# joyfang1106/MRLA

Hardware: AMD Instinct MI355X
Metric: images/sec fwd+bwd resnet50_mrlal b=256 (higher is better)
Workload: dtype bf16

## Files before the change

include/mrla_hip.h:

```cpp
#ifndef MRLA_HIP_H_
#define MRLA_HIP_H_

#include <stddef.h>
#include <stdint.h>

#ifdef __cplusplus
extern "C" {
#endif

#define MRLA_OK 0
#define MRLA_EINVAL (-1)
#define MRLA_EUNSUPPORTED (-2)
#define MRLA_EHIP (-3)

enum { MRLA_F32 = 0, MRLA_BF16 = 1, MRLA_F16 = 2 };
enum { MRLA_NCHW = 0, MRLA_NHWC = 1 };
enum { MRLA_ACT_NONE = 0, MRLA_ACT_GELU = 1 };
enum { MRLA_BN_NONE = 0, MRLA_BN_TRAIN = 1, MRLA_BN_EVAL = 2 };

#define MRLA_FWD_MOMENTS 8
#define MRLA_BWD_MOMENTS 3
#define MRLA_GEMM_MOMENTS 4

#define MRLA_ABI_VERSION 5
// ... 196 lines not shown

int mrla_conv1x1_fwd_affine_supported(int m, int k, int n, int dtype);
int mrla_conv1x1_fwd_affine(const void* x, const void* w, const float* sc, const float* sh, int relu, void* y, int m, int k,
                            int n, int dtype, void* stream);

int mrla_conv1x1_wgrad_rows(int m, int k, int n, int dtype);
int mrla_conv1x1_wgrad_plan(int m, int k, int n, int dtype, int* out);
int mrla_conv1x1_wgrad(const void* dy, const void* x, float* part, void* dw, int m, int k, int n, int dtype, int dw_dtype,
                       void* stream);

int mrla_conv1x1_wgrad_bn_supported(int m, int k, int n, int dtype);
int mrla_conv1x1_wgrad_bn(const void* g, const void* xb, const float* sc, const float* sh, const float* cb , int relu,
                          void* dy_out, const void* x, float* part, void* dw, int m, int k, int n, int dtype, int dw_dtype,
                          void* stream);

int mrla_weight_bank_refresh(const void* table, int entries, int max_tiles, void* stream);
int mrla_weight_bank_refresh_dt(const void* table, int entries, int max_tiles, int dtype, void* stream);

int mrla_reduce_rows(const float* in, float* out, int rows, int n, void* stream);
int mrla_reduce_rows2(const float* in1, float* out1, int rows1, int n1, const float* in2, float* out2, int rows2, int n2,
                      void* stream);



int mrla_light_tail_fwd(const void* x, const float* pre_sc, const float* pre_sh, const void* o_prev, const float* wq,
                        const float* wk, int ksize, const float* wv, const float* lam, const float* gamma,
                        const float* beta, float* running_mean, float* running_var, int bn_mode, float momentum, float eps,
                        const float* dp, float* mom, void* x_out, float* gate, float* bnbuf, void* out, int b, int c,
                        int h, int w, int d, int res, int fuse, int dtype, int layout, int act, void* stream);

// ... 53 lines not shown
```

mrla_amd/_lib.py:

```python
import ctypes
import os

_HERE = os.path.dirname(os.path.abspath(__file__))
LIB_PATH = os.environ.get("MRLA_HIP_LIB") or os.path.join(_HERE, "libmrla_hip.so")

ABI_VERSION = 5
OK, EINVAL, EUNSUPPORTED, EHIP = 0, -1, -2, -3
F32, BF16, F16 = 0, 1, 2
NCHW, NHWC = 0, 1
ACT_NONE, ACT_GELU = 0, 1
BN_NONE, BN_TRAIN, BN_EVAL = 0, 1, 2
FWD_MOMENTS, BWD_MOMENTS, TOKEN_PARTIALS, GEMM_MOMENTS = 8, 3, 15, 4

_ERR = {EINVAL: "invalid argument", EUNSUPPORTED: "unsupported shape/layout for the HIP kernels",
        EHIP: "HIP runtime error at kernel launch"}

_P, _I, _F = ctypes.c_void_p, ctypes.c_int, ctypes.c_float

SIGNATURES = {
    "mrla_abi_version": [],
    "mrla_light_wgrad_rows": [_I] * 6,
    "mrla_light_stats_fwd": [_P, _P, _P, _P, _I, _I, _I, _I, _I, _I, _I, _P],
    "mrla_light_gate_fwd": [_P, _P, _P, _I, _P, _I, _I, _I, _I, _P],
    "mrla_light_bn_fwd": [_P, _P, _P, _P, _P, _P, _P, _I, _F, _F, _P, _P, _P, _P, _I, _I, _I, _I, _P],
# ... 59 lines not shown
    "mrla_bn_gate_bwd": [_P, _P, _P, _P, _P, _P] + [_I] * 6 + [_P],
    "mrla_conv1x1_rows": [_I] * 4,
    "mrla_conv1x1_plan": [_I, _I, _I, _I, _I, _P],
    "mrla_conv1x1_wgrad_plan": [_I, _I, _I, _I, _P],
    "mrla_conv1x1_fwd": [_P, _P, _P, _P, _I, _I, _I, _I, _P],
    "mrla_conv1x1_add_supported": [_I] * 4,
    "mrla_conv1x1_fwd_add": [_P, _P, _P, _P, _I, _I, _I, _I, _P],
    "mrla_conv1x1_addend_supported": [_I] * 6,
    "mrla_conv1x1_fwd_addend": [_P, _P, _P, _P] + [_I] * 9 + [_P],
    "mrla_conv1x1_fwd_affine_supported": [_I] * 4,
    "mrla_conv1x1_fwd_affine": [_P, _P, _P, _P, _I, _P, _I, _I, _I, _I, _P],
    "mrla_conv1x1_wgrad_rows": [_I] * 4,
    "mrla_conv1x1_wgrad": [_P, _P, _P, _P, _I, _I, _I, _I, _I, _P],
    "mrla_conv1x1_wgrad_bn_supported": [_I] * 4,
    "mrla_conv1x1_wgrad_bn": [_P, _P, _P, _P, _P, _I, _P, _P, _P, _P, _I, _I, _I, _I, _I, _P],
    "mrla_weight_bank_refresh": [_P, _I, _I, _P],
    "mrla_weight_bank_refresh_dt": [_P, _I, _I, _I, _P],
    "mrla_reduce_rows": [_P, _P, _I, _I, _P],
    "mrla_reduce_rows2": [_P, _P, _I, _I, _P, _P, _I, _I, _P],
    "mrla_light_tail_fwd": [_P] * 6 + [_I] + [_P] * 6 + [_I, _F, _F] + [_P] * 6 + [_I] * 10 + [_P],
    "mrla_light_tail_bwd": [_P] * 5 + [_I] + [_P] * 7 + [_I] + [_P] * 5 + [_I] + [_P] * 8 + [_I] * 10 + [_P],
    "mrla_bn_fwd": [_P, _P, _I, _P, _P, _I, _P, _P, _P, _P, _I, _F, _F, _P, _I, _P] + [_I] * 6 + [_P],
    "mrla_bn_bwd": [_P] * 5 + [_I] * 4 + [_P, _P] + [_I] * 6 + [_P],
    "mrla_stem_fwd": [_P, _P, _P, _I, _P, _P, _P, _P, _I, _F, _F, _P, _P] + [_I] * 6 + [_P],
    "mrla_stem_bwd": [_P] * 5 + [_I, _I, _P, _P] + [_I] * 6 + [_P],
    "mrla_base_layer_fwd": [_P] * 6 + [_I] + [_P] * 5 + [_I, _F, _F] + [_P] * 9 + [_I] + [_P, _P] + [_I] * 9 + [_P],
    "mrla_base_layer_bwd": ([_P] * 5 + [_I] + [_P] * 6 + [_I] + [_P] * 6 + [_I] + [_P, _P] + [_I] + [_P] * 5 + [_I] + [_P] * 5
                            + [_I] * 12 + [_P]),
    "mrla_token_light_fwd": [_P] * 8 + [_I] + [_P, _P] + [_F] + [_P] * 4 + [_I] * 6 + [_P],
    "mrla_token_light_bwd": [_P] * 10 + [_I] + [_P] * 6 + [_I] + [_P] * 6 + [_I] * 6 + [_P],
# ... 52 lines not shown
```

mrla_amd/csrc/capi.hip:

```cpp
#include <algorithm>
#include <atomic>
#include <mutex>

#include "mrla_device.h"
#include "mrla_kernels.h"

namespace mrla {

hipError_t lds_opt_in(const void* kernel, size_t bytes) {
  if (bytes <= 48 * 1024) return hipSuccess;
  constexpr unsigned kSlots = 1024;
  static std::atomic<uintptr_t> keys[kSlots];
  static std::atomic<int> granted[kSlots];
  static std::mutex raise_mutex;
  int dev = 0;
  if (hipGetDevice(&dev) != hipSuccess) return hipErrorInvalidDevice;
  const uintptr_t key = reinterpret_cast<uintptr_t>(kernel) ^ ((uintptr_t)(dev + 1) << 52);
  unsigned i = (unsigned)((key >> 4) * 0x9E3779B1u) % kSlots;
  int slot = -1;
  for (unsigned probe = 0; probe < kSlots; ++probe, i = (i + 1) % kSlots) {
    uintptr_t k = keys[i].load(std::memory_order_acquire);
    if (k == 0 && keys[i].compare_exchange_strong(k, key, std::memory_order_acq_rel)) k = key;
    if (k == key) { slot = (int)i; break; }
  }
// ... 716 lines not shown

int mrla_conv1x1_wgrad_bn(const void* g, const void* xb, const float* sc, const float* sh, const float* cb, int relu,
                          void* dy_out, const void* x, float* part, void* dw, int m, int k, int n, int dtype, int dw_dtype,
                          void* stream) {
  if (!g || !xb || !sc || !sh || !cb || !dy_out || !x || !part || !dw || m <= 0 || k <= 0 || n <= 0 || bad_dtype(dtype))
    return MRLA_EINVAL;
  if (dw_dtype != MRLA_BF16 && dw_dtype != MRLA_F16 && dw_dtype != MRLA_F32) return MRLA_EINVAL;
  if ((dw_dtype == MRLA_F16 && dtype != MRLA_F16) || (dw_dtype == MRLA_BF16 && dtype == MRLA_F16)) return MRLA_EINVAL;
  if (dtype != MRLA_BF16 && dtype != MRLA_F16) return MRLA_EUNSUPPORTED;
  if (((uintptr_t)sc | (uintptr_t)sh | (uintptr_t)cb) & 15) return MRLA_EINVAL;
  if (dy_out == g || dy_out == xb) return MRLA_EINVAL;
  return launch_conv1x1_wgrad_bn(g, xb, sc, sh, cb, relu, dy_out, x, part, dw, dw_dtype == MRLA_F32, m, k, n, dtype,
                                 (hipStream_t)stream);
}

int mrla_weight_bank_refresh(const void* table, int entries, int max_tiles, void* stream) {
  if (!table || entries <= 0 || max_tiles <= 0) return MRLA_EINVAL;
  return launch_weight_bank_refresh((const long long*)table, entries, max_tiles, MRLA_BF16, (hipStream_t)stream);
}

int mrla_weight_bank_refresh_dt(const void* table, int entries, int max_tiles, int dtype, void* stream) {
  if (!table || entries <= 0 || max_tiles <= 0 || bad_dtype(dtype)) return MRLA_EINVAL;
  if (dtype != MRLA_BF16 && dtype != MRLA_F16) return MRLA_EUNSUPPORTED;
  return launch_weight_bank_refresh((const long long*)table, entries, max_tiles, dtype, (hipStream_t)stream);
}

int mrla_reduce_rows(const float* in, float* out, int rows, int n, void* stream) {
  if (!in || !out || rows <= 0 || n <= 0) return MRLA_EINVAL;
  return launch_reduce_rows(in, out, rows, n, (hipStream_t)stream);
}
// ... 71 lines not shown
```

mrla_amd/csrc/conv1x1_wgrad.hip:

```cpp
#include <algorithm>
#include <type_traits>

#include "conv1x1_elem.h"
#include "mrla_device.h"
#include "mrla_kernels.h"

namespace mrla {
namespace {

typedef short wg_s16x4 __attribute__((ext_vector_type(4)));
typedef c1_f32x16 wg_f32x16;
typedef __attribute__((address_space(3))) wg_s16x4* lds_s16x4_ptr;

constexpr int kPC = 32;
constexpr int kWgStages = 4;
constexpr int kWgWaves = 4;
#define MRLA_WG_FLAGS 0x00020000
constexpr int kWgTarget = 256;

template <int TN, int TK, int PC>
struct WgGeo {
  static constexpr int WN = (TN >= 256 && TK <= 64) ? 4 : (TK >= 256 && TN <= 64) ? 1 : 2;
  static constexpr int WK = kWgWaves / WN;
  static constexpr int WTN = TN / WN, WTK = TK / WK;
// ... 32 lines not shown
template <typename T>
__device__ __forceinline__ typename Elem16<T>::x8 frag_value(const Frag& f) {
  return __builtin_bit_cast(typename Elem16<T>::x8, __builtin_shufflevector(f.lo, f.hi, 0, 1, 2, 3, 4, 5, 6, 7));
}
__device__ __forceinline__ unsigned wg_lds_addr(const void* p) {
  return (unsigned)(size_t)((__attribute__((address_space(3))) const char*)p);
}

struct WgBnArgs {
  const void* xb;
  const float *cb, *sc, *sh;
  void* dy_out;
  int relu;
};

__device__ __forceinline__ void wg_read16(u32x4& v, unsigned addr) {
  asm volatile("ds_read_b128 %0, %1" : "=&v"(v) : "v"(addr));
}
template <int OFF>
__device__ __forceinline__ void wg_read16_at(u32x4& v, unsigned addr) {
  asm volatile("ds_read_b128 %0, %1 offset:%2" : "=&v"(v) : "v"(addr), "n"(OFF));
}
__device__ __forceinline__ void wg_write16(unsigned addr, const u32x4& v) {
  asm volatile("ds_write_b128 %0, %1" ::"v"(addr), "v"(v) : "memory");
}
__device__ __forceinline__ void wg_fence16(u32x4& v, bool wait) {
  if (wait) asm volatile("s_waitcnt lgkmcnt(0)" : "+v"(v) : : "memory");
  else asm volatile("" : "+v"(v) : : "memory");
}

template <typename T, int TN, int TK, int ST, int PC, bool BN>
__device__ __forceinline__ void conv1x1_wgrad_body(const T* __restrict__ dY, const T* __restrict__ X,
                                                   float* __restrict__ part, int M, int N, int K, int chunks_per_wg,
                                                   int nsplits, const WgBnArgs& bn) {
#if defined(__HIP_DEVICE_COMPILE__)
  typedef WgGeo<TN, TK, PC> G;
  constexpr int CPRY = TN / 8, CPRX = TK / 8;
  constexpr int SB = G::SB + (BN ? G::YB : 0);
  static_assert(G::SB < 65536, "ds offset field");
  extern __shared__ __align__(16) unsigned char smem_raw[];
  const int lane = threadIdx.x & (kWave - 1);
  const int wave = __builtin_amdgcn_readfirstlane(threadIdx.x / kWave);
  const int tiles_k = K / TK, tiles = (N / TN) * tiles_k;
  const int per = gridDim.x >> 3;
  const int vid = (blockIdx.x & 7) * per + (blockIdx.x >> 3);
  if (vid >= tiles * nsplits) return;
  const int split = vid / tiles, tile = vid - split * tiles;
  const int tn = tile / tiles_k, tk = tile - tn * tiles_k;
  const int n0 = tn * TN, k0 = tk * TK;
  const int chunks_total = (M + PC - 1) / PC;
  const int c_begin = split * chunks_per_wg;
  const int nch = min(chunks_per_wg, chunks_total - c_begin);

  const auto rsY = __builtin_amdgcn_make_buffer_rsrc(const_cast<T*>(dY), 0, (int)((size_t)M * N * 2), MRLA_WG_FLAGS);
// ... 64 lines not shown
    for (int q = 0; q < 6; ++q) {
      const float4 v = c4[q];
      cbv[4 * q] = v.x; cbv[4 * q + 1] = v.y; cbv[4 * q + 2] = v.z; cbv[4 * q + 3] = v.w;
    }
#pragma unroll
    for (int q = 0; q < 2; ++q) {
      const float4 u = s4[q], v = h4[q];
      scv[4 * q] = u.x; scv[4 * q + 1] = u.y; scv[4 * q + 2] = u.z; scv[4 * q + 3] = u.w;
      shv[4 * q] = v.x; shv[4 * q + 1] = v.y; shv[4 * q + 2] = v.z; shv[4 * q + 3] = v.w;
    }
#pragma unroll
    for (int q = 0; q < 24; ++q) asm volatile("" : "+v"(cbv[q]));
#pragma unroll
    for (int q = 0; q < 8; ++q) asm volatile("" : "+v"(scv[q]), "+v"(shv[q]));
  }
  const int relu = BN ? bn.relu : 0;
  auto rewrite = [&](unsigned sbo) {
    u32x4 gq[G::NIY], xq[G::NIY];
    const unsigned at = lds0 + sbo + wave * 1024 + lane * 16;
#pragma unroll
    for (int i = 0; i < G::NIY; ++i) {
      wg_read16(gq[i], at + i * (kWgWaves * 1024));
      wg_read16_at<G::SB>(xq[i], at + i * (kWgWaves * 1024));
    }
#pragma unroll
    for (int i = 0; i < G::NIY; ++i) {
      wg_fence16(gq[i], i == 0);
      wg_fence16(xq[i], false);
    }
#pragma unroll
// ... 5 lines not shown
      for (int w = 0; w < 4; ++w) {
        const float gv[2] = {Elem16<T>::lo(gq[i][w]), Elem16<T>::hi(gq[i][w])};
        const float xv[2] = {Elem16<T>::lo(xq[i][w]), Elem16<T>::hi(xq[i][w])};
        float y[2];
#pragma unroll
        for (int e = 0; e < 2; ++e) {
          const int j = 2 * w + e;
          const float z = fmaf(scv[j], xv[e], shv[j]);
          const float dz = (!relu || z > 0.f) ? gv[e] : 0.f;
          y[e] = fmaf(cbv[3 * j], dz, fmaf(cbv[3 * j + 1], xv[e], cbv[3 * j + 2]));
          if constexpr (!std::is_same<T, bf16_t>::value) y[e] = as_f32_result(y[e]);
        }
        o[w] = live ? Elem16<T>::pack(y[0], y[1]) : 0u;
      }
      wg_write16(at + i * (kWgWaves * 1024), o);
      __builtin_amdgcn_raw_buffer_store_b128(o, rsO, (live ? off : 0x80000000u) | skill, 0, 0);
    }
    toff += advY;
    asm volatile("s_waitcnt lgkmcnt(0)" ::: "memory");
  };

  constexpr int KSN = PC / 16, NF = 2 * (G::BN + G::BK), NI = (BN ? 2 : 1) * G::NIY + G::NIX;
  constexpr int W_NEXT = (ST - 3) * NI + (BN && ST > 3 ? G::NIY : 0);
  static_assert(KSN % 2 == 0 && ST >= 3 && W_NEXT < 64 && (ST - 2) * NI < 64, "fragment double buffer / stages / vmcnt immediate");
  Frag fa[2][G::BN], fb[2][G::BK];
  auto read_step = [&](int buf, unsigned sbo, int ks) {
#pragma unroll
    for (int i = 0; i < G::BN; ++i) frag_issue<CPRY>(fa[buf][i], offA[i] + sbo + ks * 16 * CPRY * 16);
#pragma unroll
    for (int j = 0; j < G::BK; ++j) frag_issue<CPRX>(fb[buf][j], offB[j] + sbo + ks * 16 * CPRX * 16);
  };
  auto mfma_step = [&](int buf) {
#pragma unroll
    for (int i = 0; i < G::BN; ++i)
#pragma unroll
      for (int j = 0; j < G::BK; ++j)
        Elem16<T>::mfma(acc[i][j], frag_value<T>(fa[buf][i]), frag_value<T>(fb[buf][j]));
  };
#pragma unroll
  for (int j = 0; j < ST - 1; ++j) issue(j);
  asm volatile("s_waitcnt vmcnt(%0)" ::"n"((ST - 2) * NI) : "memory");
  if constexpr (BN) rewrite(0);
  __builtin_amdgcn_s_barrier();
  asm volatile("" ::: "memory");
  read_step(0, 0, 0);
  int stage = 0, nxt = ST - 1;
  for (int c = 0; c < nch; ++c) {
    const unsigned sbo = stage * SB;
    stage = stage + 1 == ST ? 0 : stage + 1;
#pragma unroll
    for (int ks = 0; ks < KSN; ++ks) {
      const int cur = ks & 1;
      int pending = NF;
      if (ks + 1 < KSN) {
        read_step(cur ^ 1, sbo, ks + 1);
      } else if (c + 1 < nch) {
        asm volatile("s_waitcnt vmcnt(%0)" ::"n"(W_NEXT) : "memory");
        if constexpr (BN) rewrite(stage * SB);
        __builtin_amdgcn_s_barrier();
        asm volatile("" ::: "memory");
        issue(nxt);
        nxt = nxt + 1 == ST ? 0 : nxt + 1;
        read_step(0, stage * SB, 0);
      } else {
        pending = 0;
      }
#pragma unroll
      for (int i = 0; i < G::BN; ++i) {
        if (pending) frag_fence<NF>(fa[cur][i], i == 0); else frag_fence<0>(fa[cur][i], i == 0);
      }
#pragma unroll
      for (int j = 0; j < G::BK; ++j) frag_fence<0>(fb[cur][j], false);
      mfma_step(cur);
    }
  }

  float* po = part + ((size_t)split * N + n0 + wn * G::WTN) * K + k0 + wk * G::WTK + (lane & 31);
  const int h = lane >> 5;
#pragma unroll
  for (int i = 0; i < G::BN; ++i)
#pragma unroll
    for (int j = 0; j < G::BK; ++j)
#pragma unroll
      for (int e = 0; e < 16; ++e)
        po[(size_t)(i * 32 + 8 * (e >> 2) + 4 * h + (e & 3)) * K + j * 32] = acc[i][j][e];
#endif
}

template <int TN, int TK, int ST, int PC>
// ... 12 lines not shown
}
template <int TN, int TK, int ST, int PC>
__global__ __launch_bounds__(kWgWaves* kWave) void conv1x1_wgrad_bn_kernel(const bf16_t* __restrict__ g,
                                                                           const bf16_t* __restrict__ X,
                                                                           float* __restrict__ part, int M, int N, int K,
                                                                           int chunks_per_wg, int nsplits, WgBnArgs bn) {
  conv1x1_wgrad_body<bf16_t, TN, TK, ST, PC, true>(g, X, part, M, N, K, chunks_per_wg, nsplits, bn);
}
template <int TN, int TK, int ST, int PC>
__global__ __launch_bounds__(kWgWaves* kWave) void conv1x1_wgrad_bn_f16_kernel(const f16_t* __restrict__ g,
                                                                               const f16_t* __restrict__ X,
                                                                               float* __restrict__ part, int M, int N,
                                                                               int K, int chunks_per_wg, int nsplits,
                                                                               WgBnArgs bn) {
  conv1x1_wgrad_body<f16_t, TN, TK, ST, PC, true>(g, X, part, M, N, K, chunks_per_wg, nsplits, bn);
}

template <typename TO>
__device__ __forceinline__ void conv1x1_wgrad_reduce_body(const float* __restrict__ part, TO* __restrict__ dW, int splits,
                                                          int NK) {
  __shared__ float4 red[16][16];
  const int q = threadIdx.x & 15, g = threadIdx.x >> 4;
  const int e = blockIdx.x * 64 + q * 4;
  const float4* src = reinterpret_cast<const float4*>(part + e);
  const size_t pitch = (size_t)NK / 4;
  float4 a = {0.f, 0.f, 0.f, 0.f}, b = a;
  int s = g;
  for (; s + 16 < splits; s += 32) {
    const float4 u = src[(size_t)s * pitch], v = src[(size_t)(s + 16) * pitch];
    a.x += u.x; a.y += u.y; a.z += u.z; a.w += u.w;
// ... 64 lines not shown
    return MRLA_OK;
  }
  const size_t lds = (size_t)ST * G::SB;
  if (dtype == MRLA_F16) {
    if (lds_opt_in(reinterpret_cast<const void*>(conv1x1_wgrad_f16_kernel<TN, TK, ST, PC>), lds) != hipSuccess) return MRLA_EHIP;
    hipLaunchKernelGGL((conv1x1_wgrad_f16_kernel<TN, TK, ST, PC>), grid, block, lds, st, (const f16_t*)dy, (const f16_t*)x, part,
                       M, N, K, p.chunks_per_wg, p.splits);
  } else {
    if (lds_opt_in(reinterpret_cast<const void*>(conv1x1_wgrad_kernel<TN, TK, ST, PC>), lds) != hipSuccess) return MRLA_EHIP;
    hipLaunchKernelGGL((conv1x1_wgrad_kernel<TN, TK, ST, PC>), grid, block, lds, st, (const bf16_t*)dy, (const bf16_t*)x, part,
                       M, N, K, p.chunks_per_wg, p.splits);
  }
  return MRLA_OK;
}

}

int conv1x1_wgrad_rows(int M, int K, int N) {
  const WgPlan p = wgrad_plan(M, K, N);
  return p.tiles ? p.splits : MRLA_EUNSUPPORTED;
}

int conv1x1_wgrad_plan(int M, int K, int N, int* out) {
  const WgPlan p = wgrad_plan(M, K, N);
  if (!p.tiles) return MRLA_EUNSUPPORTED;
  out[0] = p.chunks_per_wg; out[1] = kWgStages; out[2] = p.tn; out[3] = p.tk; out[4] = p.splits; out[5] = p.tiles;
  return MRLA_OK;
}

int conv1x1_wgrad_bn_supported(int M, int K, int N) {
  const WgPlan p = wgrad_plan(M, K, N);
  if (!p.tiles) return MRLA_EUNSUPPORTED;
  const int ktiles = K / p.tk;
  return ktiles == 1 || (ktiles == 2 && N <= 512) ? 1 : MRLA_EUNSUPPORTED;
}

static int launch_wgrad(const void* dy, const void* x, float* part, void* dw, int dw_f32, int M, int K, int N, int dtype,
                        hipStream_t st, const WgBnArgs* bn) {
  const WgPlan p = wgrad_plan(M, K, N);
  if (!p.tiles || (dtype != MRLA_BF16 && dtype != MRLA_F16)) return MRLA_EUNSUPPORTED;
  int rc = MRLA_EUNSUPPORTED;
#define MRLA_WG_TILE(A, B) \
  if (p.tn == A && p.tk == B) rc = launch_tile<A, B, kWgStages, kPC>(p, dy, x, part, M, K, N, dtype, st, bn);
  MRLA_WG_TILE(64, 64) MRLA_WG_TILE(64, 128) MRLA_WG_TILE(64, 256) MRLA_WG_TILE(128, 64) MRLA_WG_TILE(128, 128)
  MRLA_WG_TILE(128, 256) MRLA_WG_TILE(256, 64) MRLA_WG_TILE(256, 128)
#undef MRLA_WG_TILE
  if (rc != MRLA_OK) return rc;
  const int NK = N * K;
  if (dw_f32)
    hipLaunchKernelGGL(conv1x1_wgrad_reduce_kernel<float>, dim3(NK / 64), dim3(256), 0, st, part, (float*)dw, p.splits, NK);
  else if (dtype == MRLA_F16)
    hipLaunchKernelGGL(conv1x1_wgrad_reduce_f16_kernel, dim3(NK / 64), dim3(256), 0, st, part, (f16_t*)dw, p.splits, NK);
  else
    hipLaunchKernelGGL(conv1x1_wgrad_reduce_kernel<bf16_t>, dim3(NK / 64), dim3(256), 0, st, part, (bf16_t*)dw, p.splits, NK);
  return hip_status(hipGetLastError());
}

int launch_conv1x1_wgrad(const void* dy, const void* x, float* part, void* dw, int dw_f32, int M, int K, int N, int dtype,
                         hipStream_t st) {
  return launch_wgrad(dy, x, part, dw, dw_f32, M, K, N, dtype, st, nullptr);
}

int launch_conv1x1_wgrad_bn(const void* g, const void* xb, const float* sc, const float* sh, const float* cb, int relu,
                            void* dy_out, const void* x, float* part, void* dw, int dw_f32, int M, int K, int N, int dtype,
                            hipStream_t st) {
  if (conv1x1_wgrad_bn_supported(M, K, N) != 1) return MRLA_EUNSUPPORTED;
  const WgBnArgs bn{xb, cb, sc, sh, dy_out, relu};
  return launch_wgrad(g, x, part, dw, dw_f32, M, K, N, dtype, st, &bn);
}

}
```

mrla_amd/csrc/mrla_kernels.h:

```cpp
#pragma once
#include <hip/hip_runtime.h>
#include <stddef.h>
#include <stdint.h>

#include "../../include/mrla_hip.h"

namespace mrla {

constexpr int kMaxTasksPerWave = 4;

struct SlabGeo {
  int B, C, H, W, HW;
  int CP;
  int slabs;
  int WS;
  int PW;
  int NG;
  int NB;
  int RB;
  int BG;
  int astride;
};

inline size_t dtype_size(int dtype) { return dtype == MRLA_F32 ? 4 : 2; }
// ... 156 lines not shown
int conv1x1_kstream_stages(int M, int K, int N);
int conv1x1_kstream_rows(int M, int K, int N);
int launch_conv1x1_kstream(const void* x, const void* w, void* y, float* part, int M, int K, int N, int dtype, hipStream_t st);
int launch_conv1x1_kstream_addend(const void* x, const void* w, const void* addend, void* y, int M, int K, int N, int b, int h,
                                  int wd, int sh, int sw, int dtype, hipStream_t st);
int launch_conv1x1_kstream_affine(const void* x, const void* w, const float* sc, const float* sh, int relu, void* y, int M,
                                  int K, int N, int dtype, hipStream_t st);
int conv1x1_wgrad_rows(int M, int K, int N);
int conv1x1_wgrad_plan(int M, int K, int N, int* out);
int launch_conv1x1_wgrad(const void* dy, const void* x, float* part, void* dw, int dw_f32, int M, int K, int N, int dtype,
                         hipStream_t st);
int conv1x1_wgrad_bn_supported(int M, int K, int N);
int launch_conv1x1_wgrad_bn(const void* g, const void* xb, const float* sc, const float* sh, const float* cb, int relu,
                            void* dy_out, const void* x, float* part, void* dw, int dw_f32, int M, int K, int N, int dtype,
                            hipStream_t st);
int launch_weight_bank_refresh(const long long* table, int entries, int max_tiles, int dtype, hipStream_t st);
int launch_light_stats_fwd_wide(const void* x, const void* o, const float* wv, float* mom, void* xout, const float* psc,
                                const float* psh, void* vout, int B, int C, int H, int W, int dtype, int act,
                                hipStream_t st, bool fused_no_x = false, int mom_ranges = 1);
int launch_light_apply_fwd_wide(const void* x, const void* o, const float* wv, const float* gate, const float* sc,
                                const float* sh, const float* lam, const float* dp, void* out, int B, int C, int H,
                                int W, int d, int res, int dtype, int act, hipStream_t st);
int launch_light_apply_fwd_pre_wide(const void* pre, const void* o, const float* psc, const float* psh, const float* wv,
                                    const float* gate, const float* sc, const float* sh, const float* lam,
                                    const float* dp, void* out, int B, int C, int H, int W, int d, int res, int dtype,
                                    hipStream_t st);
int launch_light_apply_bwd_wide(const void* dout, const void* x, const void* o, const float* wv, const float* gate,
                                const float* cb, const float* lam, const float* dp, const float* dyx, void* dx,
                                void* dprev, float* dwv_part, const void* pre, const float* pre_center, float* pre_tmom,
                                int B, int C, int H, int W, int d, int res, int relu, int dtype, int act, hipStream_t st);
// ... 49 lines not shown
```

mrla_amd/functional.py:

```python
import contextlib
import ctypes
import threading
import weakref
from math import log

import torch

from . import _lib as L

_DT = {torch.float32: L.F32, torch.bfloat16: L.BF16, torch.float16: L.F16}


def k_size_for(c):
    t = int(abs((log(c, 2) + 1) / 2.0))
    return t if t % 2 else t + 1


class KernelTimer:

    def __init__(self, names=None):
        self.names = None if names is None else set(names)
        self.records = []

    def summary(self):
# ... 7 lines not shown
            d["bytes_path"] += path
        return out


TIMER = None
SEQUENCES = True


LEAN = False


SHORTCUT_ADDEND = True


WGRAD_BN = True


CHANNEL_GATE = True


EVAL_FOLD = True


def _seq():
    return SEQUENCES and TIMER is None


def _seq_call(name, *args):
    L.call(name, *args)

# ... 1449 lines not shown
    def set_materialize_grads(self, flag):
        pass

    def save_for_backward(self, *tensors):
        self.saved_tensors = tensors

    def mark_non_differentiable(self, *tensors):
        pass


class _ConvBnFn(torch.autograd.Function):

    @staticmethod
    @_on_device
    def forward(ctx, x, w, gamma, beta, running_mean, running_var, training, momentum, eps, relu, defer, box, passthrough,
                w16, w16t, sub):
        ctx.set_materialize_grads(False)
        ca, cb = _SubCtx(), _SubCtx()
        res = _Conv1x1Fn.apply(x, w, bool(training), passthrough, w16, w16t, sub)
        n, k = w.shape[0], x.shape[1]
        ca.sub = tuple(sub) if (passthrough and sub is not None) else None
        ca.wshape, ca.wstride, ca.wdtype = w.shape, w.stride(), w.dtype
        ca.saved_tensors = (x, w16 if w16 is not None else w.reshape(n, k).contiguous(), w16t)
        y, part = res[0], res[1]
        out = _BnActFn.forward(cb, y, gamma, beta, running_mean, running_var, training, momentum, eps, relu, defer,
                               part if part.numel() else None, box)
        ctx.save_for_backward(*ca.saved_tensors, *cb.saved_tensors)
        ca.saved_tensors = cb.saved_tensors = ()
        ctx.ca, ctx.cb, ctx.defer, ctx.nthrough = ca, cb, bool(defer), len(res) - 2
        if defer:
            ctx.mark_non_differentiable(out[1])
            return (y, out[1]) + tuple(res[2:])
# ... 5 lines not shown
        saved = ctx.saved_tensors
        ca, cb = ctx.ca, ctx.cb
        ca.saved_tensors, cb.saved_tensors = saved[:3], saved[3:]
        try:
            return _ConvBnFn._backward(ctx, dy, rest, saved)
        finally:
            ca.saved_tensors = cb.saved_tensors = ()

    @staticmethod
    def _backward(ctx, dy, rest, saved):
        d_through = rest[-1] if ctx.nthrough else None
        ca, cb = ctx.ca, ctx.cb
        ca.needs_input_grad = (ctx.needs_input_grad[0], ctx.needs_input_grad[1])
        x, w, _ = saved[:3]
        y, gamma32, bnbuf = saved[3:]
        tail = (None,) * 12
        if dy is None:
            gx = _Conv1x1Fn.backward(ca, None, None, d_through)[0]
            return (gx, None, None, None) + tail
        n, k = w.shape
        b, _, h, wd = x.shape
        m = b * h * wd
        lib, dt = L.load(), _DT[x.dtype]
        g = dy if dy.is_contiguous(memory_format=_CL) else None
        fused = (WGRAD_BN and TIMER is None and ctx.needs_input_grad[1] and g is not None and g.dtype == y.dtype
                 and g.data_ptr() % 16 == 0 and cb.layout == L.NHWC and w.dtype == x.dtype
                 and ca.wdtype in (x.dtype, torch.float32) and lib.mrla_conv1x1_wgrad_bn_supported(m, k, n, dt) == 1)
        if not fused:
            dyc, dgamma, dbeta = _BnActFn.backward(cb, dy)[:3]
            gx, gw = _Conv1x1Fn.backward(ca, dyc, None, d_through)[:2]
            return (gx, gw, dgamma, dbeta) + tail
# ... 6 lines not shown
            tmom = torch.empty((rows, n, 2), dtype=torch.float32, device=dev)
        small = torch.empty((5, n), dtype=torch.float32, device=dev)
        mode = L.BN_TRAIN if cb.training else L.BN_EVAL
        if SEQUENCES:
            _seq_call("mrla_bn_bwd", _ptr(g), _ptr(y), _ptr(gamma32), _ptr(bnbuf), _ptr(tmom), rows, int(handed is not None),
                      mode, cb.relu, _ptr(small), None, b, n, h, wd, dt, L.NHWC, st)
        else:
            if handed is None:
                L.call("mrla_bn_plane_dmoments", _ptr(g), _ptr(y), _ptr(bnbuf[0]), _ptr(bnbuf[1]), _ptr(bnbuf[2]), cb.relu,
                       _ptr(tmom), b, n, h, wd, dt, L.NHWC, st)
            L.call("mrla_bn_stats_bwd", _ptr(tmom), _ptr(gamma32), _ptr(bnbuf[2]), _ptr(bnbuf[3]), mode, 1, _ptr(small),
                   _ptr(small[3]), _ptr(small[4]), rows, n, m // rows, st)
        prow = lib.mrla_conv1x1_wgrad_rows(m, k, n, dt)
        part = torch.empty((prow, n, k), dtype=torch.float32, device=dev)
        gw = torch.empty((n, k), dtype=ca.wdtype, device=dev)
        dyc = torch.empty_like(y)
        L.call("mrla_conv1x1_wgrad_bn", _ptr(g), _ptr(y), _ptr(bnbuf[0]), _ptr(bnbuf[1]), _ptr(small), cb.relu, _ptr(dyc),
               _ptr(x), _ptr(part), _ptr(gw), m, k, n, dt, _DT[ca.wdtype], st)
        ca.needs_input_grad = (ctx.needs_input_grad[0], False)
        gx = _Conv1x1Fn.backward(ca, dyc, None, d_through)[0]
        gw = _grad_like(gw, ca.wshape, ca.wstride)
        return (gx, gw, small[3].to(cb.gdtype), small[4].to(cb.gdtype)) + tail


def _conv_bn_fused(conv, bn, x, fused_bn):
    if not (WGRAD_BN and TIMER is None and fused_bn and torch.is_grad_enabled() and conv.weight.requires_grad):
        return False
    if x.dtype != torch.bfloat16:
        return False
    b, k, h, w = x.shape
# ... 66 lines not shown
    return tuple(downsample[0].stride)


def _gemm_weights(conv, x):
    wt, w16, w16t = conv.weight, None, None
    if wt.dtype != x.dtype:
        book = current_bookkeeping()
        held = book.bank.get(conv, x.dtype) if (book is not None and book.bank is not None and wt.dtype == torch.float32) else None
        if held is not None:
            w16, w16t = held
        else:
            wt = wt.to(x.dtype)
    return wt, w16, w16t


def conv_bn_act(x, conv, bn, relu, defer=False, passthrough=False, subsample=None, presampled=False):
    def second(t):
        return _SubsampleFn.apply(t, subsample[0], subsample[1]) if subsample is not None else t

    fused_bn = (type(bn) is torch.nn.BatchNorm2d and bn.affine and bn.track_running_stats)
    strided = (_strided_1x1(conv) and not passthrough and x.dim() == 4
               and conv1x1_applies(conv, x, "pre" if presampled else True))
    if strided or conv1x1_applies(conv, x):
        if strided and not presampled:
            x = _SubsampleFn.apply(x, conv.stride[0], conv.stride[1])
        wt, w16, w16t = _gemm_weights(conv, x)
        if _eval_fold_applies(conv, bn, x, fused_bn, defer):
            out = _conv_bn_eval_fold(x.detach(), w16 if w16 is not None else wt, bn, relu)
            return (out, second(x)) if passthrough else out
        if _conv_bn_fused(conv, bn, x, fused_bn):
            training = bn.training
            momentum = bump_batch_counter(bn) if training else bn.momentum
            box = _DeferredBnBox() if defer else None
            through = passthrough and x.requires_grad
            res = _ConvBnFn.apply(x, wt, bn.weight, bn.bias, bn.running_mean, bn.running_var, training, momentum or 0.0,
                                  bn.eps, relu, defer, box, through, w16, w16t, subsample if through else None)
            res = res if isinstance(res, tuple) else (res,)
            out = res[0]
            if defer:
                out._mrla_affine = (res[1][0], res[1][1])
                out._mrla_bn_box = box
            if not passthrough:
                return out
            return out, (res[-1] if through else second(x))
        if passthrough and torch.is_grad_enabled() and x.requires_grad:
            y, part, through = _Conv1x1Fn.apply(x, wt, bool(fused_bn and bn.training), True, w16, w16t, subsample)
            return bn_act(y, bn, relu, defer, pre_moments=part if part.numel() else None), through
        y, part = _Conv1x1Fn.apply(x, wt, bool(fused_bn and bn.training), False, w16, w16t)
        out = bn_act(y, bn, relu, defer, pre_moments=part if part.numel() else None)
        return (out, second(x)) if passthrough else out
    if presampled:
# ... 28 lines not shown
```

mrla_amd/resnet.py:

```python

import torch
import torch.nn as nn
import torch.nn.functional as F

from . import functional as F_
from . import layers


def _conv3x3(cin, cout, stride=1, groups=1, dilation=1):
    return nn.Conv2d(cin, cout, 3, stride=stride, padding=dilation, groups=groups, bias=False, dilation=dilation)


def _conv1x1(cin, cout, stride=1):
    return nn.Conv2d(cin, cout, 1, stride=stride, bias=False)


class se_layer(nn.Module):

    def __init__(self, channel, reduction=16):
        super().__init__()
        self.avg_pool = nn.AdaptiveAvgPool2d(1)
        self.fc = nn.Sequential(nn.Linear(channel, channel // reduction, bias=False), nn.ReLU(inplace=True),
                                nn.Linear(channel // reduction, channel, bias=False), nn.Sigmoid())

# ... 37 lines not shown
        self.eca = eca_layer(planes * self.expansion, int(ECA_size)) if ECA_size is not None else None
        self._norm = norm_layer

    def trunk_pre(self, x, defer_bn3=False):
        sub = F_.shortcut_subsample(self.downsample, x)
        out, identity = F_.conv_bn_act(x, self.conv1, self.bn1, relu=True, passthrough=True, subsample=sub)
        out = F_.bn_act(self.conv2(out), self.bn2, relu=True)
        if self.se is not None or self.eca is not None:
            out = F_.conv_bn_gate(out, self.conv3, self.bn3, self.se, self.eca)
        else:
            if callable(defer_bn3):
                b_, _, h_, w_ = out.shape
                cl = out.is_contiguous(memory_format=torch.channels_last) and not out.is_contiguous()
                defer_bn3 = defer_bn3(torch.empty((b_, self.conv3.out_channels, h_, w_), dtype=out.dtype, device="meta",
                                                  memory_format=torch.channels_last if cl else torch.contiguous_format))
            out = F_.conv_bn_act(out, self.conv3, self.bn3, relu=False, defer=defer_bn3)
        if self.downsample is not None:
            ds = self.downsample
            if isinstance(ds, nn.Sequential) and len(ds) == 2 and isinstance(ds[0], nn.Conv2d):
                identity = F_.conv_bn_act(identity, ds[0], ds[1], relu=False, presampled=sub is not None)
            else:
                identity = ds(identity)
        return out, identity

    def trunk(self, x):
        out, identity = self.trunk_pre(x)
        out += identity
        return self.relu(out), identity


class MRLA_Bottleneck(_BottleneckTrunk):

    def __init__(self, inplanes, planes, stride=1, downsample=None, SE=False, ECA_size=None, groups=1, base_width=64,
                 dilation=1, norm_layer=nn.BatchNorm2d, drop_path=0.0):
        super().__init__(inplanes, planes, stride, downsample, SE, ECA_size, groups, base_width, dilation, norm_layer)
# ... 258 lines not shown
```

Measured before the change: 8749.

## Fuse the 1x1 conv dX GEMM into the BN-backward wgrad kernel

After: 8933 (median of 6 runs). 1.02x the previous value.

```diff
diff --git a/include/mrla_hip.h b/include/mrla_hip.h
--- a/include/mrla_hip.h
+++ b/include/mrla_hip.h
@@ -234,6 +234,11 @@
                           void* dy_out, const void* x, float* part, void* dw, int m, int k, int n, int dtype, int dw_dtype,
                           void* stream);
 
+int mrla_conv1x1_wgrad_bn_dx_supported(int m, int k, int n, int dtype);
+int mrla_conv1x1_wgrad_bn_dx(const void* g, const void* xb, const float* sc, const float* sh, const float* cb ,
+                             int relu, const void* x, const void* wt , void* dx , float* part, void* dw,
+                             int m, int k, int n, int dtype, int dw_dtype, void* stream);
+
 int mrla_weight_bank_refresh(const void* table, int entries, int max_tiles, void* stream);
 int mrla_weight_bank_refresh_dt(const void* table, int entries, int max_tiles, int dtype, void* stream);
 
diff --git a/mrla_amd/_lib.py b/mrla_amd/_lib.py
--- a/mrla_amd/_lib.py
+++ b/mrla_amd/_lib.py
@@ -97,6 +97,8 @@
     "mrla_conv1x1_wgrad": [_P, _P, _P, _P, _I, _I, _I, _I, _I, _P],
     "mrla_conv1x1_wgrad_bn_supported": [_I] * 4,
     "mrla_conv1x1_wgrad_bn": [_P, _P, _P, _P, _P, _I, _P, _P, _P, _P, _I, _I, _I, _I, _I, _P],
+    "mrla_conv1x1_wgrad_bn_dx_supported": [_I] * 4,
+    "mrla_conv1x1_wgrad_bn_dx": [_P, _P, _P, _P, _P, _I, _P, _P, _P, _P, _P, _I, _I, _I, _I, _I, _P],
     "mrla_weight_bank_refresh": [_P, _I, _I, _P],
     "mrla_weight_bank_refresh_dt": [_P, _I, _I, _I, _P],
     "mrla_reduce_rows": [_P, _P, _I, _I, _P],
diff --git a/mrla_amd/csrc/capi.hip b/mrla_amd/csrc/capi.hip
--- a/mrla_amd/csrc/capi.hip
+++ b/mrla_amd/csrc/capi.hip
@@ -754,6 +754,26 @@
                                  (hipStream_t)stream);
 }
 
+int mrla_conv1x1_wgrad_bn_dx_supported(int m, int k, int n, int dtype) {
+  if (m <= 0 || k <= 0 || n <= 0 || bad_dtype(dtype)) return MRLA_EINVAL;
+  if (dtype != MRLA_BF16 && dtype != MRLA_F16) return MRLA_EUNSUPPORTED;
+  return conv1x1_wgrad_bn_dx_supported(m, k, n);
+}
+
+int mrla_conv1x1_wgrad_bn_dx(const void* g, const void* xb, const float* sc, const float* sh, const float* cb, int relu,
+                             const void* x, const void* wt, void* dx, float* part, void* dw, int m, int k, int n, int dtype,
+                             int dw_dtype, void* stream) {
+  if (!g || !xb || !sc || !sh || !cb || !x || !wt || !dx || !part || !dw || m <= 0 || k <= 0 || n <= 0 || bad_dtype(dtype))
+    return MRLA_EINVAL;
+  if (dw_dtype != MRLA_BF16 && dw_dtype != MRLA_F16 && dw_dtype != MRLA_F32) return MRLA_EINVAL;
+  if ((dw_dtype == MRLA_F16 && dtype != MRLA_F16) || (dw_dtype == MRLA_BF16 && dtype == MRLA_F16)) return MRLA_EINVAL;
+  if (dtype != MRLA_BF16 && dtype != MRLA_F16) return MRLA_EUNSUPPORTED;
+  if (((uintptr_t)sc | (uintptr_t)sh | (uintptr_t)cb | (uintptr_t)wt | (uintptr_t)dx) & 15) return MRLA_EINVAL;
+  if (dx == g || dx == xb || dx == x) return MRLA_EINVAL;
+  return launch_conv1x1_wgrad_bn_dx(g, xb, sc, sh, cb, relu, x, wt, dx, part, dw, dw_dtype == MRLA_F32, m, k, n, dtype,
+                                    (hipStream_t)stream);
+}
+
 int mrla_weight_bank_refresh(const void* table, int entries, int max_tiles, void* stream) {
   if (!table || entries <= 0 || max_tiles <= 0) return MRLA_EINVAL;
   return launch_weight_bank_refresh((const long long*)table, entries, max_tiles, MRLA_BF16, (hipStream_t)stream);
diff --git a/mrla_amd/csrc/conv1x1_wgrad.hip b/mrla_amd/csrc/conv1x1_wgrad.hip
--- a/mrla_amd/csrc/conv1x1_wgrad.hip
+++ b/mrla_amd/csrc/conv1x1_wgrad.hip
@@ -70,6 +70,12 @@
   int relu;
 };
 
+struct WgDxArgs {
+  const void* wt;
+  void* dx;
+};
+constexpr int kDxRowB = 64 * 2 + 16;
+
 __device__ __forceinline__ void wg_read16(u32x4& v, unsigned addr) {
   asm volatile("ds_read_b128 %0, %1" : "=&v"(v) : "v"(addr));
 }
@@ -85,15 +91,16 @@
   else asm volatile("" : "+v"(v) : : "memory");
 }
 
-template <typename T, int TN, int TK, int ST, int PC, bool BN>
+template <typename T, int TN, int TK, int ST, int PC, bool BN, bool DX = false>
 __device__ __forceinline__ void conv1x1_wgrad_body(const T* __restrict__ dY, const T* __restrict__ X,
                                                    float* __restrict__ part, int M, int N, int K, int chunks_per_wg,
-                                                   int nsplits, const WgBnArgs& bn) {
+                                                   int nsplits, const WgBnArgs& bn, const WgDxArgs& dxa = WgDxArgs{}) {
 #if defined(__HIP_DEVICE_COMPILE__)
   typedef WgGeo<TN, TK, PC> G;
   constexpr int CPRY = TN / 8, CPRX = TK / 8;
   constexpr int SB = G::SB + (BN ? G::YB : 0);
   static_assert(G::SB < 65536, "ds offset field");
+  static_assert(!DX || (BN && TN == 256 && TK == 64 && PC == 32), "the dX form: one 256 x 64 tile");
   extern __shared__ __align__(16) unsigned char smem_raw[];
   const int lane = threadIdx.x & (kWave - 1);
   const int wave = __builtin_amdgcn_readfirstlane(threadIdx.x / kWave);
@@ -188,6 +195,19 @@
 #pragma unroll
     for (int q = 0; q < 8; ++q) asm volatile("" : "+v"(scv[q]), "+v"(shv[q]));
   }
+  u32x4 wa[DX ? 16 : 1];
+  const auto rsD = __builtin_amdgcn_make_buffer_rsrc(DX ? dxa.dx : nullptr, 0, DX ? (int)((size_t)M * K * 2) : 0, MRLA_WG_FLAGS);
+  const unsigned dlimit = (unsigned)((size_t)M * K * 2);
+  const int dr = lane & 31, dh = lane >> 5, dblk = wave & 1;
+  unsigned doff = 0;
+  if constexpr (DX) {
+    const u32x4* wp = reinterpret_cast<const u32x4*>(static_cast<const T*>(dxa.wt) + (size_t)(dblk * 32 + dr) * N + dh * 8);
+#pragma unroll
+    for (int ks = 0; ks < 16; ++ks) wa[ks] = wp[ks * 2];
+#pragma unroll
+    for (int ks = 0; ks < 16; ++ks) asm volatile("" : "+v"(wa[ks]));
+    doff = (unsigned)(((size_t)c_begin * PC + wave * 8 + (lane >> 3)) * K * 2 + (lane & 7) * 16);
+  }
   const int relu = BN ? bn.relu : 0;
   auto rewrite = [&](unsigned sbo) {
     u32x4 gq[G::NIY], xq[G::NIY];
@@ -223,14 +243,54 @@
         o[w] = live ? Elem16<T>::pack(y[0], y[1]) : 0u;
       }
       wg_write16(at + i * (kWgWaves * 1024), o);
-      __builtin_amdgcn_raw_buffer_store_b128(o, rsO, (live ? off : 0x80000000u) | skill, 0, 0);
+      if constexpr (!DX) __builtin_amdgcn_raw_buffer_store_b128(o, rsO, (live ? off : 0x80000000u) | skill, 0, 0);
     }
     toff += advY;
     asm volatile("s_waitcnt lgkmcnt(0)" ::: "memory");
   };
 
+  auto dx_chunk = [&](unsigned sbo) {
+    u32x4 bq[16];
+    const unsigned rowa = lds0 + sbo + dr * (CPRY * 16);
+    const int sw = swz<CPRY>(dr);
+#pragma unroll
+    for (int ks = 0; ks < 16; ++ks) wg_read16(bq[ks], rowa + (((2 * ks + dh) ^ sw) << 4));
+#pragma unroll
+    for (int ks = 0; ks < 16; ++ks) wg_fence16(bq[ks], ks == 0);
+    wg_f32x16 d;
+#pragma unroll
+    for (int e = 0; e < 16; ++e) d[e] = 0.f;
+#pragma unroll
+    for (int ks = 0; ks < 16; ++ks)
+      Elem16<T>::mfma(d, __builtin_bit_cast(typename Elem16<T>::x8, wa[ks]), __builtin_bit_cast(typename Elem16<T>::x8, bq[ks]));
+    unsigned p[8];
+#pragma unroll
+    for (int i = 0; i < 8; ++i) p[i] = Elem16<T>::pack(d[2 * i], d[2 * i + 1]);
+#pragma unroll
+    for (int g = 0; g < 2; ++g) {
+#pragma unroll
+      for (int q = 0; q < 2; ++q) {
+        const auto sx = __builtin_amdgcn_permlane32_swap(p[4 * g + q], p[4 * g + 2 + q], false, false);
+        p[4 * g + q] = sx[0];
+        p[4 * g + 2 + q] = sx[1];
+      }
+    }
+    const unsigned to = lds0 + sbo + G::SB + dr * kDxRowB + (dblk * 32 + dh * 8) * 2;
+    wg_write16(to, (u32x4){p[0], p[1], p[2], p[3]});
+    wg_write16(to + 32, (u32x4){p[4], p[5], p[6], p[7]});
+    asm volatile("s_waitcnt lgkmcnt(0)" ::: "memory");
+  };
+  auto dx_store = [&](unsigned sbo) {
+    u32x4 v;
+    wg_read16(v, lds0 + sbo + G::SB + (wave * 8 + (lane >> 3)) * kDxRowB + (lane & 7) * 16);
+    wg_fence16(v, true);
+    __builtin_amdgcn_raw_buffer_store_b128(v, rsD, doff < dlimit ? doff : 0x80000000u, 0, 0);
+    doff += advX;
+  };
+
   constexpr int KSN = PC / 16, NF = 2 * (G::BN + G::BK), NI = (BN ? 2 : 1) * G::NIY + G::NIX;
-  constexpr int W_NEXT = (ST - 3) * NI + (BN && ST > 3 ? G::NIY : 0);
+  constexpr int W_NEXT = (ST - 3) * NI + (DX ? ST - 3 : BN && ST > 3 ? G::NIY : 0);
+  static_assert(!DX || ST == 4, "the dX form's store stream is counted for four stages");
   static_assert(KSN % 2 == 0 && ST >= 3 && W_NEXT < 64 && (ST - 2) * NI < 64, "fragment double buffer / stages / vmcnt immediate");
   Frag fa[2][G::BN], fb[2][G::BK];
   auto read_step = [&](int buf, unsigned sbo, int ks) {
@@ -252,6 +312,7 @@
   if constexpr (BN) rewrite(0);
   __builtin_amdgcn_s_barrier();
   asm volatile("" ::: "memory");
+  if constexpr (DX) __builtin_amdgcn_raw_buffer_store_b128((u32x4){0u, 0u, 0u, 0u}, rsD, 0x80000000u, 0, 0);
   read_step(0, 0, 0);
   int stage = 0, nxt = ST - 1;
   for (int c = 0; c < nch; ++c) {
@@ -268,6 +329,7 @@
         if constexpr (BN) rewrite(stage * SB);
         __builtin_amdgcn_s_barrier();
         asm volatile("" ::: "memory");
+        if constexpr (DX) dx_store(sbo);
         issue(nxt);
         nxt = nxt + 1 == ST ? 0 : nxt + 1;
         read_step(0, stage * SB, 0);
@@ -281,7 +343,15 @@
 #pragma unroll
       for (int j = 0; j < G::BK; ++j) frag_fence<0>(fb[cur][j], false);
       mfma_step(cur);
-    }
+      if constexpr (DX) {
+        if (ks == 0 && (c & 1) == (wave >> 1)) dx_chunk(sbo);
+      }
+    }
+  }
+  if constexpr (DX) {
+    __builtin_amdgcn_s_barrier();
+    asm volatile("" ::: "memory");
+    dx_store((stage == 0 ? ST - 1 : stage - 1) * SB);
   }
 
   float* po = part + ((size_t)split * N + n0 + wn * G::WTN) * K + k0 + wk * G::WTK + (lane & 31);
@@ -324,6 +394,23 @@
                                                                                int K, int chunks_per_wg, int nsplits,
                                                                                WgBnArgs bn) {
   conv1x1_wgrad_body<f16_t, TN, TK, ST, PC, true>(g, X, part, M, N, K, chunks_per_wg, nsplits, bn);
+}
+
+template <int ST>
+__global__ __launch_bounds__(kWgWaves* kWave) void conv1x1_wgrad_bn_dx_kernel(const bf16_t* __restrict__ g,
+                                                                              const bf16_t* __restrict__ X,
+                                                                              float* __restrict__ part, int M, int N, int K,
+                                                                              int chunks_per_wg, int nsplits, WgBnArgs bn,
+                                                                              WgDxArgs dxa) {
+  conv1x1_wgrad_body<bf16_t, 256, 64, ST, kPC, true, true>(g, X, part, M, N, K, chunks_per_wg, nsplits, bn, dxa);
+}
+template <int ST>
+__global__ __launch_bounds__(kWgWaves* kWave) void conv1x1_wgrad_bn_dx_f16_kernel(const f16_t* __restrict__ g,
+                                                                                  const f16_t* __restrict__ X,
+                                                                                  float* __restrict__ part, int M, int N,
+                                                                                  int K, int chunks_per_wg, int nsplits,
+                                                                                  WgBnArgs bn, WgDxArgs dxa) {
+  conv1x1_wgrad_body<f16_t, 256, 64, ST, kPC, true, true>(g, X, part, M, N, K, chunks_per_wg, nsplits, bn, dxa);
 }
 
 template <typename TO>
@@ -418,6 +505,24 @@
   return MRLA_OK;
 }
 
+int launch_tile_dx(const WgPlan& p, const void* g, const void* x, float* part, int M, int K, int N, int dtype, hipStream_t st,
+                   const WgBnArgs& bn, const WgDxArgs& dxa) {
+  typedef WgGeo<256, 64, kPC> G;
+  const dim3 grid((p.tiles * p.splits + 7) / 8 * 8), block(kWgWaves * kWave);
+  constexpr size_t lds = (size_t)kWgStages * (G::SB + G::YB);
+  static_assert(lds <= 160 * 1024 && kPC * kDxRowB <= G::YB, "LDS of a CU / the staging tile inside the xb tile");
+  if (dtype == MRLA_F16) {
+    if (lds_opt_in(reinterpret_cast<const void*>(conv1x1_wgrad_bn_dx_f16_kernel<kWgStages>), lds) != hipSuccess) return MRLA_EHIP;
+    hipLaunchKernelGGL((conv1x1_wgrad_bn_dx_f16_kernel<kWgStages>), grid, block, lds, st, (const f16_t*)g, (const f16_t*)x, part, M,
+                       N, K, p.chunks_per_wg, p.splits, bn, dxa);
+  } else {
+    if (lds_opt_in(reinterpret_cast<const void*>(conv1x1_wgrad_bn_dx_kernel<kWgStages>), lds) != hipSuccess) return MRLA_EHIP;
+    hipLaunchKernelGGL((conv1x1_wgrad_bn_dx_kernel<kWgStages>), grid, block, lds, st, (const bf16_t*)g, (const bf16_t*)x, part, M,
+                       N, K, p.chunks_per_wg, p.splits, bn, dxa);
+  }
+  return MRLA_OK;
+}
+
 }
 
 int conv1x1_wgrad_rows(int M, int K, int N) {
@@ -439,16 +544,27 @@
   return ktiles == 1 || (ktiles == 2 && N <= 512) ? 1 : MRLA_EUNSUPPORTED;
 }
 
+int conv1x1_wgrad_bn_dx_supported(int M, int K, int N) {
+  if (conv1x1_wgrad_bn_supported(M, K, N) != 1) return MRLA_EUNSUPPORTED;
+  const WgPlan p = wgrad_plan(M, K, N);
+  return p.tiles == 1 && p.tn == 256 && p.tk == 64 ? 1 : MRLA_EUNSUPPORTED;
+}
+
 static int launch_wgrad(const void* dy, const void* x, float* part, void* dw, int dw_f32, int M, int K, int N, int dtype,
-                        hipStream_t st, const WgBnArgs* bn) {
+                        hipStream_t st, const WgBnArgs* bn, const WgDxArgs* dxa = nullptr) {
   const WgPlan p = wgrad_plan(M, K, N);
   if (!p.tiles || (dtype != MRLA_BF16 && dtype != MRLA_F16)) return MRLA_EUNSUPPORTED;
   int rc = MRLA_EUNSUPPORTED;
+  if (dxa) {
+    if (!bn || conv1x1_wgrad_bn_dx_supported(M, K, N) != 1) return MRLA_EUNSUPPORTED;
+    rc = launch_tile_dx(p, dy, x, part, M, K, N, dtype, st, *bn, *dxa);
+  } else {
 #define MRLA_WG_TILE(A, B) \
   if (p.tn == A && p.tk == B) rc = launch_tile<A, B, kWgStages, kPC>(p, dy, x, part, M, K, N, dtype, st, bn);
-  MRLA_WG_TILE(64, 64) MRLA_WG_TILE(64, 128) MRLA_WG_TILE(64, 256) MRLA_WG_TILE(128, 64) MRLA_WG_TILE(128, 128)
-  MRLA_WG_TILE(128, 256) MRLA_WG_TILE(256, 64) MRLA_WG_TILE(256, 128)
+    MRLA_WG_TILE(64, 64) MRLA_WG_TILE(64, 128) MRLA_WG_TILE(64, 256) MRLA_WG_TILE(128, 64) MRLA_WG_TILE(128, 128)
+    MRLA_WG_TILE(128, 256) MRLA_WG_TILE(256, 64) MRLA_WG_TILE(256, 128)
 #undef MRLA_WG_TILE
+  }
   if (rc != MRLA_OK) return rc;
   const int NK = N * K;
   if (dw_f32)
@@ -473,4 +589,13 @@
   return launch_wgrad(g, x, part, dw, dw_f32, M, K, N, dtype, st, &bn);
 }
 
-}
+int launch_conv1x1_wgrad_bn_dx(const void* g, const void* xb, const float* sc, const float* sh, const float* cb, int relu,
+                               const void* x, const void* wt, void* dx, float* part, void* dw, int dw_f32, int M, int K, int N,
+                               int dtype, hipStream_t st) {
+  if (conv1x1_wgrad_bn_dx_supported(M, K, N) != 1) return MRLA_EUNSUPPORTED;
+  const WgBnArgs bn{xb, cb, sc, sh, nullptr, relu};
+  const WgDxArgs dxa{wt, dx};
+  return launch_wgrad(g, x, part, dw, dw_f32, M, K, N, dtype, st, &bn, &dxa);
+}
+
+}
diff --git a/mrla_amd/csrc/mrla_kernels.h b/mrla_amd/csrc/mrla_kernels.h
--- a/mrla_amd/csrc/mrla_kernels.h
+++ b/mrla_amd/csrc/mrla_kernels.h
@@ -194,6 +194,10 @@
 int launch_conv1x1_wgrad_bn(const void* g, const void* xb, const float* sc, const float* sh, const float* cb, int relu,
                             void* dy_out, const void* x, float* part, void* dw, int dw_f32, int M, int K, int N, int dtype,
                             hipStream_t st);
+int conv1x1_wgrad_bn_dx_supported(int M, int K, int N);
+int launch_conv1x1_wgrad_bn_dx(const void* g, const void* xb, const float* sc, const float* sh, const float* cb, int relu,
+                               const void* x, const void* wt, void* dx, float* part, void* dw, int dw_f32, int M, int K, int N,
+                               int dtype, hipStream_t st);
 int launch_weight_bank_refresh(const long long* table, int entries, int max_tiles, int dtype, hipStream_t st);
 int launch_light_stats_fwd_wide(const void* x, const void* o, const float* wv, float* mom, void* xout, const float* psc,
                                 const float* psh, void* vout, int B, int C, int H, int W, int dtype, int act,
diff --git a/mrla_amd/functional.py b/mrla_amd/functional.py
--- a/mrla_amd/functional.py
+++ b/mrla_amd/functional.py
@@ -45,6 +45,9 @@
 
 
 WGRAD_BN = True
+
+
+WGRAD_BN_DX = True
 
 
 CHANNEL_GATE = True
@@ -1524,8 +1527,9 @@
     @staticmethod
     @_on_device
     def forward(ctx, x, w, gamma, beta, running_mean, running_var, training, momentum, eps, relu, defer, box, passthrough,
-                w16, w16t, sub):
+                w16, w16t, sub, fuse_dx=False):
         ctx.set_materialize_grads(False)
+        ctx.fuse_dx = bool(fuse_dx)
         ca, cb = _SubCtx(), _SubCtx()
         res = _Conv1x1Fn.apply(x, w, bool(training), passthrough, w16, w16t, sub)
         n, k = w.shape[0], x.shape[1]
@@ -1561,7 +1565,7 @@
         ca.needs_input_grad = (ctx.needs_input_grad[0], ctx.needs_input_grad[1])
         x, w, _ = saved[:3]
         y, gamma32, bnbuf = saved[3:]
-        tail = (None,) * 12
+        tail = (None,) * 13
         if dy is None:
             gx = _Conv1x1Fn.backward(ca, None, None, d_through)[0]
             return (gx, None, None, None) + tail
@@ -1598,6 +1602,15 @@
         prow = lib.mrla_conv1x1_wgrad_rows(m, k, n, dt)
         part = torch.empty((prow, n, k), dtype=torch.float32, device=dev)
         gw = torch.empty((n, k), dtype=ca.wdtype, device=dev)
+        if (WGRAD_BN_DX and ctx.fuse_dx and ctx.needs_input_grad[0] and d_through is None and ca.sub is None
+                and lib.mrla_conv1x1_wgrad_bn_dx_supported(m, k, n, dt) == 1):
+            w16t = saved[2]
+            wt = w16t if w16t is not None else w.t().contiguous()
+            gx = torch.empty_like(x)
+            L.call("mrla_conv1x1_wgrad_bn_dx", _ptr(g), _ptr(y), _ptr(bnbuf[0]), _ptr(bnbuf[1]), _ptr(small), cb.relu, _ptr(x),
+                   _ptr(wt), _ptr(gx), _ptr(part), _ptr(gw), m, k, n, dt, _DT[ca.wdtype], st)
+            gw = _grad_like(gw, ca.wshape, ca.wstride)
+            return (gx, gw, small[3].to(cb.gdtype), small[4].to(cb.gdtype)) + tail
         dyc = torch.empty_like(y)
         L.call("mrla_conv1x1_wgrad_bn", _ptr(g), _ptr(y), _ptr(bnbuf[0]), _ptr(bnbuf[1]), _ptr(small), cb.relu, _ptr(dyc),
                _ptr(x), _ptr(part), _ptr(gw), m, k, n, dt, _DT[ca.wdtype], st)
@@ -1694,7 +1707,7 @@
     return wt, w16, w16t
 
 
-def conv_bn_act(x, conv, bn, relu, defer=False, passthrough=False, subsample=None, presampled=False):
+def conv_bn_act(x, conv, bn, relu, defer=False, passthrough=False, subsample=None, presampled=False, fuse_dx=False):
     def second(t):
         return _SubsampleFn.apply(t, subsample[0], subsample[1]) if subsample is not None else t
 
@@ -1714,7 +1727,7 @@
             box = _DeferredBnBox() if defer else None
             through = passthrough and x.requires_grad
             res = _ConvBnFn.apply(x, wt, bn.weight, bn.bias, bn.running_mean, bn.running_var, training, momentum or 0.0,
-                                  bn.eps, relu, defer, box, through, w16, w16t, subsample if through else None)
+                                  bn.eps, relu, defer, box, through, w16, w16t, subsample if through else None, fuse_dx)
             res = res if isinstance(res, tuple) else (res,)
             out = res[0]
             if defer:
diff --git a/mrla_amd/resnet.py b/mrla_amd/resnet.py
--- a/mrla_amd/resnet.py
+++ b/mrla_amd/resnet.py
@@ -75,11 +75,11 @@
                 cl = out.is_contiguous(memory_format=torch.channels_last) and not out.is_contiguous()
                 defer_bn3 = defer_bn3(torch.empty((b_, self.conv3.out_channels, h_, w_), dtype=out.dtype, device="meta",
                                                   memory_format=torch.channels_last if cl else torch.contiguous_format))
-            out = F_.conv_bn_act(out, self.conv3, self.bn3, relu=False, defer=defer_bn3)
+            out = F_.conv_bn_act(out, self.conv3, self.bn3, relu=False, defer=defer_bn3, fuse_dx=True)
         if self.downsample is not None:
             ds = self.downsample
             if isinstance(ds, nn.Sequential) and len(ds) == 2 and isinstance(ds[0], nn.Conv2d):
-                identity = F_.conv_bn_act(identity, ds[0], ds[1], relu=False, presampled=sub is not None)
+                identity = F_.conv_bn_act(identity, ds[0], ds[1], relu=False, presampled=sub is not None, fuse_dx=True)
             else:
                 identity = ds(identity)
         return out, identity
```
